# MatrixPlayer/face_alignment_cvpr_2012

Measured on NVIDIA B200. Metric: face crops/sec (head pose + 10-pt FFD), higher is better.
Workload: dtype f32+int32

## Files before the change

face_alignment_cvpr_2012_b200/csrc/device_forest.h:

```cpp
#pragma once
#include <cstdint>
#include <string>
#include <vector>

#include "model.h"

namespace crf {

constexpr int kRowStride = 128;
typedef uint32_t stack_t;
constexpr bool kStack16 = sizeof(stack_t) == 2;
constexpr int kStripArea = kStack16 ? 257 : (1 << 20);
constexpr uint32_t kSumMask = kStack16 ? 0xffffu : 0xffffffffu;
constexpr int kPatch = 31;
constexpr int kHalfPatch = 15;
constexpr int kParts = 10;
constexpr int kMaxList = 128;

struct alignas(32) DevSlot {
  uint16_t a1;
  uint8_t w1, ns1;
  uint16_t hs1;
  uint16_t hl1;
  uint16_t a2;
// ... 5 lines not shown
  uint32_t m1, m2;
  int32_t child;
};
static_assert(sizeof(DevSlot) == 32, "slot must be one 32-byte sector");

struct alignas(16) DevSlot16 { uint32_t r1, r2; int32_t child; uint32_t areas; };
static_assert(sizeof(DevSlot16) == 16, "compact slot is 16 bytes");

constexpr int kWinTile = 8;
constexpr int kWinExtent = 30;
constexpr int kWinRows = kWinTile + kWinExtent;
constexpr int kWinCols = 40;
constexpr int kWinRowBytes = kWinCols * 4;
constexpr int kWinPlaneBytes = kWinRows * kWinRowBytes;
struct alignas(32) DevSlotW {
  uint32_t px1, px2;
  uint32_t yh1, yh2;
  uint32_t m1, m2;
  int32_t child;
  uint32_t tw;
};
static_assert(sizeof(DevSlotW) == 32, "window slot is one 32-byte sector");

struct alignas(32) DevSlotN {
  uint32_t pw1, pw2;
  uint32_t yh1, yh2;
  uint32_t m1, m2;
  int32_t left_thr;
  int32_t right;
};
static_assert(sizeof(DevSlotN) == 32, "internal-node slot is one 32-byte sector");
constexpr int kSlotNChildBits = 22;

struct alignas(16) DevMpLeaf {
  int16_t off[kParts][2];
  float weight;
  uint32_t pad;
};
static_assert(sizeof(DevMpLeaf) == 48, "leaf record is three 16-byte words");

struct PackedForest {
  std::vector<DevSlot> slots;
  std::vector<DevSlot16> slots16;
  std::vector<DevSlotW> slotsw;
  std::vector<DevSlotN> slotsn;
  std::vector<int32_t> nroot;
  int max_extent = 0;
  std::vector<int32_t> roots;
  std::vector<int32_t> forest_base;
  std::vector<int32_t> forest_ntrees;
  std::vector<int32_t> leaf_base;
  std::vector<int32_t> leaf_oid;
  std::vector<float> hp_m;
  std::vector<DevMpLeaf> mp_leaf;
  std::vector<uint16_t> mp_mask;
  int max_depth = 0;
};

struct PackOptions {
  float hp_min_foreground = 0.5f;
  int ffd_min_samples = 2;
  float ffd_min_foreground = 0.5f;
  float ffd_min_pf = 0.25f;
  float ffd_max_variance = 25.f;
};

int pack_forests(const std::vector<const FlatForest*>& forests, ForestKind kind, const PackOptions& opt, PackedForest& out, std::string& err);

inline uint32_t magic_for_area(uint32_t area) { return (uint32_t)((1ull << 31) / area) + 1u; }

}
```

face_alignment_cvpr_2012_b200/csrc/engine.cu:

```cuda
#include <algorithm>
#include <atomic>
#include <cmath>
#include <cstdio>
#include <cstdlib>
#include <cstring>
#include <memory>
#include <sstream>
#include <string>
#include <thread>
#include <unordered_map>
#include <vector>

#include "kernels.cuh"
#include "model.h"

struct crf_model { crf::Model m; };

namespace crf {

thread_local std::string g_last_error;
static int fail(int code, const std::string& msg) { g_last_error = msg; return code; }

#define CU(call)                                                                                          \
  do {                                                                                                    \
// ... 94 lines not shown
};
static ChannelLayout layout_of(const std::vector<int>& sorted_features) {
  ChannelLayout L;
  auto plain = [&](int which) { L.pp.which[L.n_plain] = which; L.pp.plane[L.n_plain] = L.nplanes++; L.n_plain++; };
  for (int f : sorted_features) {
    switch (f) {
      case 0: plain(0); break;
      case 1: L.gabor_first = L.nplanes; L.nplanes += 35; break;
      case 2: plain(1); plain(2); break;
      case 3: plain(3); plain(4); break;
      case 4: plain(6); L.canny = true; break;
      case 5: plain(5); break;
      default: break;
    }
  }
  return L;
}

}

using namespace crf;

struct crf_ctx {
  int device = 0;
  cudaStream_t copy_stream = nullptr;
  cudaEvent_t ev_copied[2] = {nullptr, nullptr}, ev_consumed[2] = {nullptr, nullptr};
  uint8_t* h_stage[2] = {nullptr, nullptr};
  size_t h_stage_bytes[2] = {0, 0};
  crf_options_t opt{};
  int hp_ntrees = 0, mp_ntrees_cfg = 0, num_channels = 38;
  ChannelLayout layout;
  bool full_model = true;
  PackedForest hp, mp;
  Buf d_hp_slotsn, d_mp_slotsn, d_hp_nroot, d_mp_nroot, d_hp_slotsw, d_mp_slotsw, d_hp_slots16, d_mp_slots16, d_hp_slots, d_hp_roots, d_hp_m, d_mp_slots, d_mp_roots, d_mp_mask, d_mp_leaf, d_xs, d_coef[5], d_coef_sep[5];
  int gabor_width[5] = {0, 0, 0, 0, 0};
  ComposeTables ct{};
  struct WorkSet {
    cudaStream_t stream = nullptr;
    Buf d_gabor_scratch, d_gabor_counters;
    Buf d_scaled, d_stacks, d_mag, d_minmax, d_hp_leaf, d_ffd_leaf, d_face_roots, d_face_ntrees, d_votes, d_vote_counts, d_vote_base, d_seg_counts, d_u8planes, d_int32;
    size_t scaled_fs = 0, stack_fs = 0, plane_stride = 0, mag_fs = 0, mag_ps = 0, hp_leaf_fs = 0, ffd_leaf_fs = 0, vote_cap = 0, u8_fs = 0;
    Buf* all[16] = {&d_gabor_scratch, &d_gabor_counters, &d_scaled, &d_stacks, &d_mag, &d_minmax, &d_hp_leaf, &d_ffd_leaf, &d_face_roots, &d_face_ntrees, &d_votes, &d_vote_counts, &d_vote_base,
                    &d_seg_counts, &d_u8planes, &d_int32};
  };
  WorkSet ws[2];
  WorkSet* w = &ws[0];
  Buf d_imgs[2], d_fd, d_faces, d_counters, d_misc;
  crf_counters_t cnt{};
  bool counting = false;
  int traverse_variant = 0;
  int sm_count = 148;
  int win_hp = 0, win_ffd = 0;
  bool win_smem_ok = true;
  int win_tex = 1;
  cudaTextureObject_t tex_hp = 0, tex_mp = 0, tex_hp_wide = 0, tex_mp_wide = 0, tex_hp_n = 0, tex_mp_n = 0;
  int win_fmt = 2;
  int nstreams = 1;
  int gabor_fused = 0;
  int gabor_band = 32;
  int gabor_quant_old = 0;
  int ms_mode = CRF_MS_FAST;
  int ms_variant = 3;
  size_t work_budget = (size_t)64 << 30;
  StageTimer timer;
  unsigned long long haar_cached = 0;
  Buf d_haar_stages, d_haar_weak, d_haar_feats, d_haar_nodes, d_haar_leaves, d_haar_tilt, d_haar_T, d_haar_frames, d_haar_S, d_haar_Q, d_haar_flags, d_haar_list[2], d_haar_rows, d_haar_levels, d_haar_counts, d_haar_cand;
  std::vector<int> haar_split{3, 8};
// ... 294 lines not shown

static int launch_meanshift(crf_ctx* c, const FaceDesc* fd, int nchains, crf_face_t* faces) {
  Span s(c, CRF_STAGE_MEANSHIFT);
  MeanShiftOpt mo{c->opt.ms_kernel_size, c->opt.ms_max_iterations, c->opt.ms_stopping_criteria};
  const int cpc = nchains >= 8192 ? 32 : std::max(1, std::min(8, nchains / 296));
  const dim3 grid((nchains + cpc - 1) / cpc);
  unsigned long long* cnt = c->counting ? c->d_counters.as<unsigned long long>() : nullptr;
  if (c->ms_mode == CRF_MS_FAST) {
    const bool dense = c->w->ffd_leaf_fs >= 65536 || c->w->vote_cap >= 65536;
    if (dense) k_meanshift_fast<512><<<nchains, 512, 0, c->w->stream>>>(fd, nchains, c->w->d_votes.as<DevVote>(), c->w->vote_cap, c->w->d_vote_counts.as<int32_t>(),
                                                                       c->w->d_vote_base.as<int32_t>(), mo, faces, cnt);
    else k_meanshift_fast<128><<<nchains, 128, 0, c->w->stream>>>(fd, nchains, c->w->d_votes.as<DevVote>(), c->w->vote_cap, c->w->d_vote_counts.as<int32_t>(),
                                                                 c->w->d_vote_base.as<int32_t>(), mo, faces, cnt);
    KCHECK(); count_launch(c, CRF_STAGE_MEANSHIFT);
    return CRF_OK;
  }
#define CRF_MS(MINB)                                                                                                                                    \
  k_meanshift<MINB, false><<<grid, kFoldThreads, MsGeom<false>::smem, c->w->stream>>>(fd, nchains, c->w->d_votes.as<DevVote>(), c->w->vote_cap, c->w->d_vote_counts.as<int32_t>(), \
                                                                  c->w->d_vote_base.as<int32_t>(), cpc, mo, faces, cnt)
  if (cpc < 32)
    k_meanshift<3, true><<<grid, kFoldThreads, MsGeom<true>::smem, c->w->stream>>>(fd, nchains, c->w->d_votes.as<DevVote>(), c->w->vote_cap, c->w->d_vote_counts.as<int32_t>(),
                                                                     c->w->d_vote_base.as<int32_t>(), cpc, mo, faces, cnt);
  else if (c->ms_variant == 2) CRF_MS(2); else if (c->ms_variant == 4) CRF_MS(4); else CRF_MS(3);
#undef CRF_MS
  KCHECK(); count_launch(c, CRF_STAGE_MEANSHIFT);
  return CRF_OK;
}

static int launch_votes_meanshift(crf_ctx* c, const FaceDesc* fd, int n, int stride, crf_face_t* faces) {
  {
    Span s(c, CRF_STAGE_VOTES);
    VoteArgs a{};
    a.fd = fd; a.leaf_ids = c->w->d_ffd_leaf.as<int32_t>(); a.leaf_face_stride = c->w->ffd_leaf_fs; a.face_ntrees = c->w->d_face_ntrees.as<int32_t>(); a.stride = stride;
    a.mp_mask = c->d_mp_mask.as<uint16_t>(); a.mp_leaf = c->d_mp_leaf.as<DevMpLeaf>(); a.votes = c->w->d_votes.as<DevVote>(); a.vote_cap = c->w->vote_cap;
    a.seg_counts = c->w->d_seg_counts.as<int32_t>(); a.vote_counts = c->w->d_vote_counts.as<int32_t>(); a.vote_base = c->w->d_vote_base.as<int32_t>(); a.faces = faces;
    CU(cudaMemsetAsync(a.vote_counts, 0, (size_t)n * kParts * 4, c->w->stream));
    k_votes_count<<<dim3(kVoteSegs / 8, n), 256, 0, c->w->stream>>>(a);
    KCHECK();
    k_votes_offsets<<<(n + 127) / 128, 128, 0, c->w->stream>>>(a, n);
    KCHECK();
    k_votes_emit<<<dim3(kVoteSegs / 8, n), 256, 0, c->w->stream>>>(a);
    KCHECK(); count_launch(c, CRF_STAGE_VOTES, 3);
  }
  return launch_meanshift(c, fd, n * kParts, faces);
}

static int run_faces(crf_ctx* c, const FaceDesc* d_fd, int n, int Hmax, const uint8_t* d_imgs, crf_face_t* d_faces, bool headpose_only, int tree_cap,
                     cudaEvent_t imgs_consumed) {
  int rc;
  if ((rc = launch_resize(c, d_fd, n, Hmax, d_imgs))) return rc;
  if (imgs_consumed) CU(cudaEventRecord(imgs_consumed, c->w->stream));
  if ((rc = launch_channels(c, d_fd, n, Hmax, c->layout, false))) return rc;
  if ((rc = launch_traverse(c, d_fd, n, Hmax, true, c->opt.hp_stride, c->d_hp_roots.as<int32_t>(), c->hp_ntrees, c->hp_ntrees, true))) return rc;
  if ((rc = launch_hp_reduce(c, d_fd, n, c->opt.hp_stride, !headpose_only, tree_cap, d_faces))) return rc;
  if (headpose_only) return CRF_OK;
  if ((rc = launch_traverse(c, d_fd, n, Hmax, false, c->opt.ffd_stride, nullptr, 0, tree_cap))) return rc;
  if ((rc = launch_votes_meanshift(c, d_fd, n, c->opt.ffd_stride, d_faces))) return rc;
  return CRF_OK;
}

static int pick_chunk(const crf_ctx* c, int Hmax, bool headpose_only) {
  const size_t np_hp = (size_t)patches_1d(125, c->opt.hp_stride) * patches_1d(Hmax, c->opt.hp_stride);
  const size_t np_ffd = headpose_only ? 0 : (size_t)patches_1d(125, c->opt.ffd_stride) * patches_1d(Hmax, c->opt.ffd_stride);
  const size_t per_face = (size_t)Hmax * 128 + (size_t)(Hmax + 1) * kRowStride * sizeof(stack_t) * c->layout.nplanes +
                          (c->layout.gabor_first >= 0 && !c->gabor_fused ? (size_t)Hmax * 128 * 4 * 35 + 35 * 2 * 4 : 0) + np_hp * c->hp_ntrees * 4 +
                          np_ffd * c->mp_ntrees_cfg * (4 + 3 * sizeof(DevVote)) + (size_t)kMaxList * 4 + 4 +
                          (headpose_only ? 0 : (size_t)kVoteSegs * kParts * 4 + 2 * kParts * 4) + sizeof(FaceDesc) + sizeof(crf_face_t);
// ... 757 lines not shown
    PackedForest pf;
    std::vector<const FlatForest*> fs;
    if (which == 0) fs.push_back(&m->m.hp); else for (auto& f : m->m.jungle) fs.push_back(&f);
    const int rc = pack_forests(fs, which == 0 ? KIND_HEADPOSE : KIND_MULTIPART, po, pf, err);
    if (rc) return fail(rc, err);
    if (pf.slots.size() != pf.slots16.size() || pf.slots.size() != pf.slotsw.size()) return fail(CRF_ERR_STATE, "record arrays differ in length");
    int ext = 0;
    for (size_t i = 0; i < pf.slots.size(); i++) {
      const DevSlot& a = pf.slots[i]; const DevSlot16& b = pf.slots16[i]; const DevSlotW& w = pf.slotsw[i];
      const bool leaf16 = (b.r1 >> 26) & 1u, leafw = (w.tw >> 31) & 1u;
      if ((a.is_leaf != 0) != leaf16 || leaf16 != leafw) return fail(CRF_ERR_STATE, "leaf flags disagree");
      if (a.is_leaf) {
        if (b.child != a.child || (int32_t)w.m2 != a.child || w.child != (int32_t)i || (w.tw & 0xffffu) != 0x7fffu || w.px1 || w.px2 || w.yh1 || w.yh2 || w.m1)
          return fail(CRF_ERR_STATE, "leaf record mismatch");
      } else {
        const int x1 = a.a1 % kRowStride, y1 = a.a1 / kRowStride, x2 = a.a2 % kRowStride, y2 = a.a2 / kRowStride;
        const int h1 = ((a.ns1 - 1) * a.hs1 + a.hl1) / kRowStride, h2 = ((a.ns2 - 1) * a.hs2 + a.hl2) / kRowStride;
        const bool ok16 = (int)(b.r1 & 31) == x1 && (int)((b.r1 >> 5) & 31) == y1 && (int)((b.r1 >> 10) & 31) == a.w1 && (int)((b.r1 >> 15) & 31) == h1 &&
                          (int)((b.r1 >> 20) & 63) == a.ch && (int)(b.r2 & 31) == x2 && (int)((b.r2 >> 5) & 31) == y2 && (int)((b.r2 >> 10) & 31) == a.w2 &&
                          (int)((b.r2 >> 15) & 31) == h2 && (int)((b.r2 >> 20) & 0x3ff) - 256 == a.thr && b.child == a.child &&
                          (b.areas & 0xffff) == (uint32_t)a.w1 * h1 && (b.areas >> 16) == (uint32_t)a.w2 * h2;
        const bool okw = w.px1 == (uint32_t)a.ch * kWinPlaneBytes + x1 * 4u && w.px2 == (uint32_t)a.ch * kWinPlaneBytes + x2 * 4u &&
                         w.yh1 == ((uint32_t)y1 * kWinRowBytes | ((uint32_t)h1 * kWinRowBytes) << 16) && w.yh2 == ((uint32_t)y2 * kWinRowBytes | ((uint32_t)h2 * kWinRowBytes) << 16) &&
                         w.m1 == a.m1 && w.m2 == a.m2 && w.child == a.child && (int)(short)(w.tw & 0xffffu) == a.thr &&
                         ((w.tw >> 16) & 0xffu) == a.w1 * 4u && ((w.tw >> 24) & 0x7fu) == a.w2 * 4u &&
                         a.m1 == magic_for_area((uint32_t)a.w1 * h1) && a.m2 == magic_for_area((uint32_t)a.w2 * h2);
        if (!ok16 || !okw) return fail(CRF_ERR_STATE, "record forms disagree at slot " + std::to_string(i));
        if (a.child <= (int32_t)i || (size_t)a.child + 1 >= pf.slots.size()) return fail(CRF_ERR_STATE, "children are not laid out after their parent");
        ext = std::max(ext, std::max(std::max(x1 + a.w1, y1 + h1), std::max(x2 + a.w2, y2 + h2)));
      }
      checked++;
    }
    if (ext != pf.max_extent) return fail(CRF_ERR_STATE, "max_extent is not the largest rectangle extent");
    if (!pf.nroot.empty()) {
      if (pf.nroot.size() != pf.roots.size()) return fail(CRF_ERR_STATE, "nroot and roots differ in length");
      std::vector<std::pair<int32_t, int32_t>> st;
      for (size_t t = 0; t < pf.roots.size(); t++) {
        st.assign(1, {pf.roots[t], pf.nroot[t]});
        while (!st.empty()) {
          const auto [si, ni] = st.back(); st.pop_back();
          const DevSlot& a = pf.slots[si];
          if (a.is_leaf) { if (ni != ~a.child) return fail(CRF_ERR_STATE, "DevSlotN leaf tag mismatch"); continue; }
          if (ni < 0 || (size_t)ni >= pf.slotsn.size()) return fail(CRF_ERR_STATE, "DevSlotN index out of range");
          const DevSlotN& r = pf.slotsn[ni]; const DevSlotW& w = pf.slotsw[si];
          const int32_t left = (int32_t)((uint32_t)r.left_thr << (32 - kSlotNChildBits)) >> (32 - kSlotNChildBits), thr = r.left_thr >> kSlotNChildBits;
          if ((r.pw1 & 0x3ffffu) != w.px1 || (r.pw2 & 0x3ffffu) != w.px2 || (r.pw1 >> 18) != ((w.tw >> 16) & 0xffu) || (r.pw2 >> 18) != ((w.tw >> 24) & 0x7fu) ||
              r.yh1 != w.yh1 || r.yh2 != w.yh2 || r.m1 != w.m1 || r.m2 != w.m2 || thr != std::min(255, std::max(-256, (int)a.thr)))
            return fail(CRF_ERR_STATE, "DevSlotN test mismatch at slot " + std::to_string(si));
          st.push_back({a.child, left});
          st.push_back({a.child + 1, r.right});
        }
      }
    }
    if (which == 0 && max_extent_hp) *max_extent_hp = ext;
    if (which == 1 && max_extent_ffd) *max_extent_ffd = ext;
  }
  return (int)std::min<long long>(checked, 0x7fffffff);
}

void crf_model_free(crf_model* m) { delete m; }

int crf_device_count(void) {
  int n = 0;
  if (cudaGetDeviceCount(&n) != cudaSuccess) { cudaGetLastError(); return 0; }
  return n;
}

void crf_ctx_destroy(crf_ctx* c) {
  if (!c) return;
  cudaSetDevice(c->device);
  for (auto& w : c->ws) if (w.stream) cudaStreamSynchronize(w.stream);
  if (c->tex_hp) cudaDestroyTextureObject(c->tex_hp);
  if (c->tex_mp) cudaDestroyTextureObject(c->tex_mp);
  if (c->tex_hp_n) cudaDestroyTextureObject(c->tex_hp_n);
  if (c->tex_mp_n) cudaDestroyTextureObject(c->tex_mp_n);
  if (c->tex_hp_wide) cudaDestroyTextureObject(c->tex_hp_wide);
  if (c->tex_mp_wide) cudaDestroyTextureObject(c->tex_mp_wide);
  Buf* all[] = {&c->d_hp_slotsn, &c->d_mp_slotsn, &c->d_hp_nroot, &c->d_mp_nroot, &c->d_hp_slotsw, &c->d_mp_slotsw, &c->d_hp_slots16, &c->d_mp_slots16, &c->d_hp_slots, &c->d_hp_roots, &c->d_hp_m, &c->d_mp_slots, &c->d_mp_roots, &c->d_mp_mask, &c->d_mp_leaf, &c->d_xs, &c->d_coef[0], &c->d_coef[1],
                &c->d_coef[2], &c->d_coef[3], &c->d_coef[4], &c->d_coef_sep[1], &c->d_coef_sep[2], &c->d_coef_sep[3], &c->d_coef_sep[4], &c->d_imgs[0], &c->d_imgs[1], &c->d_fd, &c->d_faces, &c->d_counters, &c->d_misc,
                &c->d_haar_stages, &c->d_haar_weak, &c->d_haar_feats, &c->d_haar_nodes, &c->d_haar_leaves, &c->d_haar_tilt, &c->d_haar_T, &c->d_haar_frames, &c->d_haar_S, &c->d_haar_Q, &c->d_haar_flags, &c->d_haar_list[0],
                &c->d_haar_list[1], &c->d_haar_rows, &c->d_haar_levels, &c->d_haar_counts, &c->d_haar_cand};
  for (Buf* b : all) b->release();
  for (auto& w : c->ws) {
    for (Buf* b : w.all) b->release();
    if (w.stream) cudaStreamDestroy(w.stream);
  }
  c->timer.destroy();
  for (int i = 0; i < 2; i++) { if (c->ev_copied[i]) cudaEventDestroy(c->ev_copied[i]); if (c->ev_consumed[i]) cudaEventDestroy(c->ev_consumed[i]); }
  if (c->copy_stream) cudaStreamDestroy(c->copy_stream);
  for (int i = 0; i < 2; i++) if (c->h_stage[i]) cudaFreeHost(c->h_stage[i]);
  delete c;
}

int crf_ctx_create(const crf_model* m, int device, const crf_options_t* opt, crf_ctx** out) {
  if (!out) return fail(CRF_ERR_ARG, "null argument");
  *out = nullptr;
  static const crf_model no_forests = [] { crf_model e; e.m.features = {0, 1, 2}; e.m.num_channels = 38; return e; }();
  if (!m) m = &no_forests;
  int ndev = 0;
  if (cudaGetDeviceCount(&ndev) != cudaSuccess || ndev <= 0) { cudaGetLastError(); return fail(CRF_ERR_CUDA, "no CUDA device: this library has no CPU fallback"); }
  if (device < 0 || device >= ndev) return fail(CRF_ERR_ARG, "device index out of range");
  const bool full = !m->m.hp.trees.empty() && m->m.jungle.size() == CRF_NUM_POSE_FORESTS;
  if (!m->m.hp.trees.empty() && !m->m.jungle.empty() && m->m.jungle.size() != CRF_NUM_POSE_FORESTS)
    return fail(CRF_ERR_UNSUPPORTED, "the facial-feature jungle must hold 5 pose forests (src/FaceForest.cpp:216-222)");
  CU(cudaSetDevice(device));
  crf_ctx* c = new crf_ctx();
  struct Guard { crf_ctx* c; ~Guard() { if (c) crf_ctx_destroy(c); } } guard{c};
  c->device = device;
  if (opt) c->opt = *opt; else crf_options_default(&c->opt);
  if (c->opt.hp_stride < 1 || c->opt.ffd_stride < 1) return fail(CRF_ERR_ARG, "strides must be >= 1");
  if (const char* v = std::getenv("CRF_TRAVERSE_VARIANT")) c->traverse_variant = (int)std::strtol(v, nullptr, 0);
// ... 21 lines not shown
  }
  for (auto& w : c->ws) CU(cudaStreamCreateWithFlags(&w.stream, cudaStreamNonBlocking));
  CU(cudaStreamCreateWithFlags(&c->copy_stream, cudaStreamNonBlocking));
  for (int i = 0; i < 2; i++) {
    CU(cudaEventCreateWithFlags(&c->ev_copied[i], cudaEventDisableTiming));
    CU(cudaEventCreateWithFlags(&c->ev_consumed[i], cudaEventDisableTiming));
  }
  PackOptions po;
  po.hp_min_foreground = c->opt.hp_min_foreground; po.ffd_min_samples = c->opt.ffd_min_samples; po.ffd_min_foreground = c->opt.ffd_min_foreground;
  po.ffd_min_pf = c->opt.ffd_min_pf; po.ffd_max_variance = c->opt.ffd_max_variance;
  std::string err;
  int rc = CRF_OK;
  if (!m->m.hp.trees.empty() && (rc = pack_forests({&m->m.hp}, KIND_HEADPOSE, po, c->hp, err))) return fail(rc, err);
  std::vector<const FlatForest*> jf;
  for (auto& f : m->m.jungle) jf.push_back(&f);
  if (!jf.empty() && (rc = pack_forests(jf, KIND_MULTIPART, po, c->mp, err))) return fail(rc, err);
  c->hp_ntrees = (int)c->hp.roots.size();
  c->mp_ntrees_cfg = std::max(m->m.mp_ntrees_cfg, 1);
  c->num_channels = m->m.num_channels;
  c->full_model = full;
  c->layout = layout_of(std::vector<int>(m->m.features.begin(), m->m.features.end()));
  if (c->layout.nplanes != c->num_channels) return fail(CRF_ERR_STATE, "feature list and plane count disagree");
  if (c->hp_ntrees > kMaxList || c->mp_ntrees_cfg > kMaxList) return fail(CRF_ERR_UNSUPPORTED, "forest size outside 1..128 trees");
  if ((rc = upload(c->d_hp_slots16, c->hp.slots16, c->w->stream)) || (rc = upload(c->d_mp_slots16, c->mp.slots16, c->w->stream))) return rc;
  if ((rc = upload(c->d_hp_slotsw, c->hp.slotsw, c->w->stream)) || (rc = upload(c->d_mp_slotsw, c->mp.slotsw, c->w->stream))) return rc;
  CU(cudaDeviceGetAttribute(&c->sm_count, cudaDevAttrMultiProcessorCount, device));
  {
    int optin = 0;
    CU(cudaDeviceGetAttribute(&optin, cudaDevAttrMaxSharedMemoryPerBlockOptin, device));
    c->win_smem_ok = optin >= kWinSmemBytes;
  }
  if ((rc = upload(c->d_hp_slots, c->hp.slots, c->w->stream)) || (rc = upload(c->d_hp_roots, c->hp.roots, c->w->stream)) || (rc = upload(c->d_hp_m, c->hp.hp_m, c->w->stream)) ||
      (rc = upload(c->d_mp_slots, c->mp.slots, c->w->stream)) || (rc = upload(c->d_mp_roots, c->mp.roots, c->w->stream)) ||
      (rc = upload(c->d_mp_mask, c->mp.mp_mask, c->w->stream)) || (rc = upload(c->d_mp_leaf, c->mp.mp_leaf, c->w->stream)))
    return rc;
  for (int k = 0; k < 2; k++) {
    const PackedForest& pf = k ? c->mp : c->hp;
    if (pf.slotsn.empty() && pf.nroot.empty()) continue;
    std::vector<int32_t> map(pf.slots.size(), -1);
    for (size_t t = 0; t < pf.roots.size(); t++) map[pf.roots[t]] = pf.nroot[t];
    std::vector<DevSlotN> recs = pf.slotsn;
    if (recs.empty()) recs.emplace_back();
    if ((rc = upload(k ? c->d_mp_slotsn : c->d_hp_slotsn, recs, c->w->stream)) || (rc = upload(k ? c->d_mp_nroot : c->d_hp_nroot, map, c->w->stream))) return rc;
  }
  for (int k = 0; k < 6; k++) {
    cudaResourceDesc rd{}; rd.resType = cudaResourceTypeLinear;
    void* ptrs[6] = {c->d_hp_slotsw.p, c->d_mp_slotsw.p, c->d_hp_slots.p, c->d_mp_slots.p, c->d_hp_slotsn.p, c->d_mp_slotsn.p};
    const size_t counts[6] = {c->hp.slotsw.size(), c->mp.slotsw.size(), c->hp.slots.size(), c->mp.slots.size(),
                              c->d_hp_slotsn.p ? std::max<size_t>(c->hp.slotsn.size(), 1) : 0, c->d_mp_slotsn.p ? std::max<size_t>(c->mp.slotsn.size(), 1) : 0};
    cudaTextureObject_t* objs[6] = {&c->tex_hp, &c->tex_mp, &c->tex_hp_wide, &c->tex_mp_wide, &c->tex_hp_n, &c->tex_mp_n};
    if (counts[k] == 0) continue;
    rd.res.linear.devPtr = ptrs[k];
    rd.res.linear.desc = cudaCreateChannelDesc<uint4>();
    rd.res.linear.sizeInBytes = counts[k] * 32;
    cudaTextureDesc td{}; td.readMode = cudaReadModeElementType;
    CU(cudaCreateTextureObject(objs[k], &rd, &td, nullptr));
  }
  {
    float poseT[6];
    poseT[0] = -2.5; poseT[1] = -0.35; poseT[2] = -0.20; poseT[3] = -poseT[2]; poseT[4] = -poseT[1]; poseT[5] = -poseT[0];
    std::vector<double> xs;
    for (int j = 0; j < 5; j++) {
      c->ct.bin_begin[j] = (int)xs.size();
      const double step = 0.01;
      for (double x = poseT[j]; x < poseT[j + 1]; x += step) xs.push_back(x);
    }
    c->ct.bin_begin[5] = (int)xs.size();
// ... 665 lines not shown
```

face_alignment_cvpr_2012_b200/csrc/kernels.cuh:

```cuda
#pragma once
#include <cuda_runtime.h>
#include <stdint.h>

#include "../../include/crf_b200.h"
#include "device_forest.h"

namespace crf {

struct FaceDesc {
  unsigned long long img_off;
  unsigned long long img_step;
  int bx, by, bw, bh;
  int W, H;
  float scale;
  int pad;
  double scale_x, scale_y;
};

enum { CNT_HP_TESTS = 0, CNT_FFD_TESTS, CNT_HP_TRAV, CNT_FFD_TRAV, CNT_VOTES, CNT_VOTE_PASSES, CNT_NUM };

__device__ __forceinline__ int border101(int p, int len) {
  if (len == 1) return 0;
  while (p < 0 || p >= len) p = p < 0 ? -p : 2 * len - 2 - p;
  return p;
// ... 1601 lines not shown
    for (int j = warp; j < kFoldChains && f0 + j < nfaces; j += kFoldThreads / 32)
      compose_face(s_mean[j], s_var[j], ct, lane, faces + f0 + j, face_roots + (size_t)(f0 + j) * kMaxList, face_ntrees + f0 + j);
}

__global__ void k_area_under_curve(float x1, float x2, double mean, double sd, float* out) {
  double sum = 0;
  const double step = 0.01;
  for (double x = x1; x < x2; x += step) {
    const double t = (x - mean) / sd;
    sum += exp(-0.5 * (t * t)) * step;
  }
  *out = (float)(sum * 1.0 / (sd * sqrt(2 * 3.14159265358979323846)));
}

__global__ void k_compose_only(float headpose, float variance, ComposeTables ct, crf_face_t* face, int32_t* list, int32_t* ntrees) {
  compose_face(headpose, variance, ct, threadIdx.x & 31, face, list, ntrees);
}

__global__ void __launch_bounds__(288) k_compose_batch(const float* __restrict__ headpose, const float* __restrict__ variance, int n, ComposeTables ct,
                                                       crf_face_t* __restrict__ faces, int32_t* __restrict__ lists, int32_t* __restrict__ ntrees) {
  const int i = blockIdx.x * 9 + (threadIdx.x >> 5);
  if (i >= n) return;
  compose_face(headpose[i], variance[i], ct, threadIdx.x & 31, faces + i, lists + (size_t)i * kMaxList, ntrees + i);
}

struct __align__(8) DevVote { short x, y; float w; };

constexpr int kVoteSegs = 128;

struct VoteArgs {
  const FaceDesc* fd;
  const int32_t* leaf_ids; size_t leaf_face_stride;
  const int32_t* face_ntrees; int stride;
  const uint16_t* mp_mask; const DevMpLeaf* mp_leaf;
  DevVote* votes; size_t vote_cap;
  int32_t* seg_counts;
  int32_t* vote_counts;
  int32_t* vote_base;
  crf_face_t* faces;
};

__device__ __forceinline__ void vote_segment(const VoteArgs& a, int f, int seg, int& n, int& k0, int& k1, int& nt, int& ny) {
  const FaceDesc d = a.fd[f];
  nt = a.face_ntrees[f];
  const int nx = (d.W - kPatch + a.stride - 1) / a.stride;
  ny = (d.H - kPatch + a.stride - 1) / a.stride;
  n = max(nx, 0) * max(ny, 0) * nt;
  const int per = (((n + kVoteSegs - 1) / kVoteSegs) + 31) & ~31;
  k0 = min(n, seg * per);
  k1 = min(n, k0 + per);
}

__global__ void __launch_bounds__(256) k_votes_count(VoteArgs a) {
  const int f = blockIdx.y, lane = threadIdx.x & 31, seg = blockIdx.x * 8 + (threadIdx.x >> 5);
  int n, k0, k1, nt, ny;
  vote_segment(a, f, seg, n, k0, k1, nt, ny);
  const int32_t* __restrict__ ids = a.leaf_ids + f * a.leaf_face_stride;
  auto spread5 = [](unsigned x) { return (x * 0x108421u) & 0x01041041u; };
  unsigned lo = 0, hi = 0;
  const bool swar = (k1 - k0 + 31) / 32 <= 63;
  int cnt = 0;
  for (int kb = k0; kb < k1; kb += 128) {
    int id[4];
    unsigned mask[4];
#pragma unroll
    for (int u = 0; u < 4; u++) { const int k = kb + u * 32 + lane; id[u] = k < k1 ? ids[k] : -1; }
#pragma unroll
    for (int u = 0; u < 4; u++) mask[u] = id[u] >= 0 ? (unsigned)__ldg(a.mp_mask + id[u]) : 0u;
    if (swar) {
#pragma unroll
      for (int u = 0; u < 4; u++) { lo += spread5(mask[u] & 31u); hi += spread5(mask[u] >> 5); }
    } else {
#pragma unroll
      for (int p = 0; p < kParts; p++) {
        int c = 0;
#pragma unroll
        for (int u = 0; u < 4; u++) c += __popc(__ballot_sync(0xffffffffu, (mask[u] >> p) & 1u));
        if (lane == p) cnt += c;
      }
    }
  }
  if (swar) {
#pragma unroll
    for (int p = 0; p < kParts; p++) {
      const int c = (int)__reduce_add_sync(0xffffffffu, ((p < 5 ? lo : hi) >> (6 * (p % 5))) & 63u);
      if (lane == p) cnt = c;
    }
  }
  if (lane < kParts) {
    a.seg_counts[((size_t)f * kVoteSegs + seg) * kParts + lane] = cnt;
    if (cnt) atomicAdd(&a.vote_counts[f * kParts + lane], cnt);
  }
}

__global__ void k_votes_offsets(VoteArgs a, int nfaces) {
  const int f = blockIdx.x * blockDim.x + threadIdx.x;
  if (f >= nfaces) return;
  long long run = 0;
  for (int p = 0; p < kParts; p++) { a.vote_base[f * kParts + p] = (int32_t)run; run += a.vote_counts[f * kParts + p]; }
  if (run > (long long)a.vote_cap) {
    for (int p = 0; p < kParts; p++) { a.vote_base[f * kParts + p] = 0; a.vote_counts[f * kParts + p] = -1; }
    a.faces[f].flags |= 4;
  }
}

__global__ void __launch_bounds__(256) k_votes_emit(VoteArgs a) {
  const int f = blockIdx.y, lane = threadIdx.x & 31, seg = blockIdx.x * 8 + (threadIdx.x >> 5);
  int n, k0, k1, nt, ny;
  vote_segment(a, f, seg, n, k0, k1, nt, ny);
  if (k0 >= k1 || a.vote_counts[f * kParts] < 0) return;
  int base[kParts];
  const int32_t* sc = a.seg_counts + (size_t)f * kVoteSegs * kParts;
#pragma unroll
  for (int p = 0; p < kParts; p++) {
    int v = 0;
    for (int s = lane; s < seg; s += 32) v += sc[s * kParts + p];
    base[p] = __reduce_add_sync(0xffffffffu, v) + a.vote_base[f * kParts + p];
  }
  const int32_t* __restrict__ ids = a.leaf_ids + f * a.leaf_face_stride;
  DevVote* __restrict__ fv = a.votes + (size_t)f * a.vote_cap;
  const unsigned m_nt = 0xffffffffu / (unsigned)nt + 1u, m_ny = 0xffffffffu / (unsigned)max(ny, 1) + 1u;
  int leaf_n = 0;
  unsigned mask_n = 0;
  if (k0 + lane < k1) { leaf_n = ids[k0 + lane]; mask_n = __ldg(a.mp_mask + leaf_n); }
  auto spread5 = [](unsigned x) { return (x * 0x108421u) & 0x01041041u; };
  for (int k = k0 + lane; k - lane < k1; k += 32) {
    const int leaf = leaf_n;
    const unsigned mask = mask_n;
    leaf_n = 0; mask_n = 0;
    if (k + 32 < k1) { leaf_n = ids[k + 32]; mask_n = __ldg(a.mp_mask + leaf_n); }
    const unsigned own_lo = spread5(mask & 31u), own_hi = spread5(mask >> 5);
    unsigned lo = own_lo, hi = own_hi;
#pragma unroll
    for (int o = 1; o < 32; o <<= 1) {
      const unsigned nl = __shfl_up_sync(0xffffffffu, lo, o), nh = __shfl_up_sync(0xffffffffu, hi, o);
      if (lane >= o) { lo += nl; hi += nh; }
    }
    const unsigned tot_lo = __shfl_sync(0xffffffffu, lo, 31), tot_hi = __shfl_sync(0xffffffffu, hi, 31);
    if (mask) {
      const unsigned ex_lo = lo - own_lo, ex_hi = hi - own_hi;
      const int patch = nt == 1 ? k : (int)__umulhi((unsigned)k, m_nt);
      const int ix = ny == 1 ? patch : (int)__umulhi((unsigned)patch, m_ny), iy = patch - ix * ny;
      const int cx = ix * a.stride + kHalfPatch, cy = iy * a.stride + kHalfPatch;
      union { uint4 q[3]; DevMpLeaf L; } u;
      const uint4* lp = reinterpret_cast<const uint4*>(a.mp_leaf + leaf);
      u.q[0] = __ldg(lp); u.q[1] = __ldg(lp + 1); u.q[2] = __ldg(lp + 2);
      const DevMpLeaf& L = u.L;
#pragma unroll
      for (int p = 0; p < kParts; p++) {
        if ((mask >> p) & 1u) {
          DevVote v;
          v.x = (short)(L.off[p][0] + cx);
          v.y = (short)(L.off[p][1] + cy);
          v.w = L.weight;
          fv[base[p] + (int)(((p < 5 ? ex_lo : ex_hi) >> (6 * (p % 5))) & 63u)] = v;
        }
      }
    }
#pragma unroll
    for (int p = 0; p < kParts; p++) base[p] += (int)(((p < 5 ? tot_lo : tot_hi) >> (6 * (p % 5))) & 63u);
  }
}

struct MeanShiftOpt { int kernel; int max_iterations; float stopping; };

struct ExpfTable { unsigned long long tab[32]; };
__constant__ ExpfTable c_expf;

__device__ __forceinline__ float expf_glibc(float x, const unsigned long long* __restrict__ tab) {
  const double N = 32.0;
  const double InvLn2N = 0x1.71547652b82fep+0 * N;
  const double C0 = 0x1.c6af84b912394p-5 / N / N / N, C1 = 0x1.ebfce50fac4f3p-3 / N / N, C2 = 0x1.62e42ff0c52d6p-1 / N;
  const double xd = (double)x;
  if (!(xd > -103.0)) return xd != xd ? x : 0.f;
  if (xd > 88.0) return __int_as_float(0x7f800000);
  const double z = InvLn2N * xd;
  const double kd = rint(z);
  const long long ki = (long long)kd;
  const double r = z - kd;
  const double s = __longlong_as_double((long long)(tab[ki & 31] + ((unsigned long long)ki << 47)));
  const double zz = fma(C0, r, C1);
  const double r2 = r * r;
  double y = fma(C2, r, 1.0);
  y = fma(zz, r2, y);
  return (float)(y * s);
}

__device__ __forceinline__ void vote_terms(const DevVote q, bool first_pass, float mx, float my, float lamda, const unsigned long long* __restrict__ tab,
                                           float& w, float& wx, float& wy) {
  if (first_pass) {
    w = q.w;
  } else {
    const float dx = mx - (float)q.x, dy = my - (float)q.y;
// ... 231 lines not shown
```

face_alignment_cvpr_2012_b200/csrc/pack.cc:

```cpp
#include <algorithm>
#include <deque>

#include "../../include/crf_b200.h"
#include "device_forest.h"

namespace crf {

int pack_forests(const std::vector<const FlatForest*>& forests, ForestKind kind, const PackOptions& opt, PackedForest& out, std::string& err) {
  out = PackedForest();
  for (const FlatForest* f : forests) {
    out.forest_base.push_back((int32_t)out.roots.size());
    out.forest_ntrees.push_back((int32_t)f->trees.size());
    for (const FlatTree& t : f->trees) {
      if (t.nodes.empty()) { err = "empty tree"; return CRF_ERR_FORMAT; }
      const int32_t leaf_base = (int32_t)out.leaf_oid.size();
      out.leaf_base.push_back(leaf_base);
      out.max_depth = t.max_depth > out.max_depth ? t.max_depth : out.max_depth;
      const size_t nleaves = kind == KIND_HEADPOSE ? t.hp_leaves.size() : t.mp_leaves.size();
      out.leaf_oid.resize(leaf_base + nleaves);
      if (kind == KIND_HEADPOSE) {
        out.hp_m.resize(leaf_base + nleaves);
        for (size_t l = 0; l < nleaves; l++) {
          const HpLeaf& L = t.hp_leaves[l];
          out.leaf_oid[leaf_base + l] = L.object_id;
          float m = -1.f;
          if (L.foreground > opt.hp_min_foreground) {
            m = 0;
            for (int j = 0; j < 5; j++) m += L.labels[j] * j;
            m /= (L.nsamples * L.foreground);
            if (!(m >= 0.f)) m = __builtin_nanf("");
          }
          out.hp_m[leaf_base + l] = m;
        }
      } else {
        out.mp_leaf.resize(leaf_base + nleaves);
        out.mp_mask.resize(leaf_base + nleaves);
        for (size_t l = 0; l < nleaves; l++) {
          const MpLeaf& L = t.mp_leaves[l];
          out.leaf_oid[leaf_base + l] = L.object_id;
          DevMpLeaf d{};
          uint16_t mask = 0;
          for (int i = 0; i < kParts; i++) {
            if (L.offset[i][0] < -32768 || L.offset[i][0] > 32767 || L.offset[i][1] < -32768 || L.offset[i][1] > 32767) {
              err = "leaf offset does not fit int16"; return CRF_ERR_UNSUPPORTED;
            }
            d.off[i][0] = (int16_t)L.offset[i][0];
            d.off[i][1] = (int16_t)L.offset[i][1];
            float min_pf = opt.ffd_min_pf;
            if (i == 0 || i == 7) min_pf *= 1.5;
            if (L.foreground > opt.ffd_min_foreground && L.prob_foreground[i] > min_pf && L.variance[i] < opt.ffd_max_variance &&
                L.samples > opt.ffd_min_samples)
              mask |= (uint16_t)(1u << i);
          }
          d.weight = L.foreground;
          out.mp_leaf[leaf_base + l] = d;
          out.mp_mask[leaf_base + l] = mask;
        }
      }
      const int32_t base = (int32_t)out.slots.size();
      out.roots.push_back(base);
      std::vector<int32_t> slot_of(t.nodes.size(), -1);
      std::vector<int32_t> n_of(t.nodes.size(), 0);
      auto tag = [&](int32_t ni) {
        if (t.nodes[ni].leaf >= 0) n_of[ni] = ~(leaf_base + t.nodes[ni].leaf);
        else { n_of[ni] = (int32_t)out.slotsn.size(); out.slotsn.emplace_back(); }
      };
      tag(0);
      out.nroot.push_back(n_of[0]);
      std::deque<int32_t> q;
      out.slots.emplace_back();
      slot_of[0] = base;
      q.push_back(0);
      while (!q.empty()) {
        const int32_t ni = q.front();
        q.pop_front();
        const FlatNode& n = t.nodes[ni];
        DevSlot s{};
        if (n.leaf >= 0) {
          s.is_leaf = 1;
          s.child = leaf_base + n.leaf;
        } else {
          if (n.left < 0 || n.right < 0 || n.left >= (int32_t)t.nodes.size() || n.right >= (int32_t)t.nodes.size()) { err = "dangling child"; return CRF_ERR_FORMAT; }
          const int32_t pair = (int32_t)out.slots.size();
          out.slots.emplace_back();
          out.slots.emplace_back();
          slot_of[n.left] = pair;
          slot_of[n.right] = pair + 1;
          q.push_back(n.left);
          q.push_back(n.right);
// ... 71 lines not shown
```

Baseline: 42310.

## Repack vote leaves and compact vote emission through shared-memory owner map

New measurement: 42780 (median of 6 runs). +1.1%, better.

```diff
diff --git a/face_alignment_cvpr_2012_b200/csrc/device_forest.h b/face_alignment_cvpr_2012_b200/csrc/device_forest.h
--- a/face_alignment_cvpr_2012_b200/csrc/device_forest.h
+++ b/face_alignment_cvpr_2012_b200/csrc/device_forest.h
@@ -61,12 +61,11 @@
 static_assert(sizeof(DevSlotN) == 32, "internal-node slot is one 32-byte sector");
 constexpr int kSlotNChildBits = 22;
 
-struct alignas(16) DevMpLeaf {
-  int16_t off[kParts][2];
+struct alignas(8) DevVoteLeaf {
+  uint32_t mask;
   float weight;
-  uint32_t pad;
 };
-static_assert(sizeof(DevMpLeaf) == 48, "leaf record is three 16-byte words");
+static_assert(sizeof(DevVoteLeaf) == 8, "vote leaf record is one 64-bit load");
 
 struct PackedForest {
   std::vector<DevSlot> slots;
@@ -81,8 +80,8 @@
   std::vector<int32_t> leaf_base;
   std::vector<int32_t> leaf_oid;
   std::vector<float> hp_m;
-  std::vector<DevMpLeaf> mp_leaf;
-  std::vector<uint16_t> mp_mask;
+  std::vector<DevVoteLeaf> mp_leaf;
+  std::vector<uint32_t> mp_off;
   int max_depth = 0;
 };
 
diff --git a/face_alignment_cvpr_2012_b200/csrc/engine.cu b/face_alignment_cvpr_2012_b200/csrc/engine.cu
--- a/face_alignment_cvpr_2012_b200/csrc/engine.cu
+++ b/face_alignment_cvpr_2012_b200/csrc/engine.cu
@@ -150,7 +150,7 @@
   ChannelLayout layout;
   bool full_model = true;
   PackedForest hp, mp;
-  Buf d_hp_slotsn, d_mp_slotsn, d_hp_nroot, d_mp_nroot, d_hp_slotsw, d_mp_slotsw, d_hp_slots16, d_mp_slots16, d_hp_slots, d_hp_roots, d_hp_m, d_mp_slots, d_mp_roots, d_mp_mask, d_mp_leaf, d_xs, d_coef[5], d_coef_sep[5];
+  Buf d_hp_slotsn, d_mp_slotsn, d_hp_nroot, d_mp_nroot, d_hp_slotsw, d_mp_slotsw, d_hp_slots16, d_mp_slots16, d_hp_slots, d_hp_roots, d_hp_m, d_mp_slots, d_mp_roots, d_mp_leaf, d_mp_off, d_xs, d_coef[5], d_coef_sep[5];
   int gabor_width[5] = {0, 0, 0, 0, 0};
   ComposeTables ct{};
   struct WorkSet {
@@ -511,7 +511,7 @@
     Span s(c, CRF_STAGE_VOTES);
     VoteArgs a{};
     a.fd = fd; a.leaf_ids = c->w->d_ffd_leaf.as<int32_t>(); a.leaf_face_stride = c->w->ffd_leaf_fs; a.face_ntrees = c->w->d_face_ntrees.as<int32_t>(); a.stride = stride;
-    a.mp_mask = c->d_mp_mask.as<uint16_t>(); a.mp_leaf = c->d_mp_leaf.as<DevMpLeaf>(); a.votes = c->w->d_votes.as<DevVote>(); a.vote_cap = c->w->vote_cap;
+    a.mp_leaf = c->d_mp_leaf.as<DevVoteLeaf>(); a.mp_off = c->d_mp_off.as<uint32_t>(); a.votes = c->w->d_votes.as<DevVote>(); a.vote_cap = c->w->vote_cap;
     a.seg_counts = c->w->d_seg_counts.as<int32_t>(); a.vote_counts = c->w->d_vote_counts.as<int32_t>(); a.vote_base = c->w->d_vote_base.as<int32_t>(); a.faces = faces;
     CU(cudaMemsetAsync(a.vote_counts, 0, (size_t)n * kParts * 4, c->w->stream));
     k_votes_count<<<dim3(kVoteSegs / 8, n), 256, 0, c->w->stream>>>(a);
@@ -1335,6 +1335,23 @@
       checked++;
     }
     if (ext != pf.max_extent) return fail(CRF_ERR_STATE, "max_extent is not the largest rectangle extent");
+    if (which == 1) {
+      size_t l = 0;
+      for (const FlatForest* f : fs)
+        for (const FlatTree& t : f->trees)
+          for (const MpLeaf& L : t.mp_leaves) {
+            if (l >= pf.mp_leaf.size() || pf.mp_off.size() != pf.mp_leaf.size() * kParts)
+              return fail(CRF_ERR_STATE, "vote tables differ in length from the leaves");
+            for (int i = 0; i < kParts; i++) {
+              const uint32_t o = pf.mp_off[l * kParts + i];
+              if ((int16_t)(o & 0xffffu) != L.offset[i][0] || (int16_t)(o >> 16) != L.offset[i][1])
+                return fail(CRF_ERR_STATE, "vote offset mismatch at leaf " + std::to_string(l));
+            }
+            if (std::memcmp(&pf.mp_leaf[l].weight, &L.foreground, sizeof(float)) != 0) return fail(CRF_ERR_STATE, "vote weight mismatch at leaf " + std::to_string(l));
+            l++;
+          }
+      if (l != pf.mp_leaf.size()) return fail(CRF_ERR_STATE, "vote tables differ in length from the leaves");
+    }
     if (!pf.nroot.empty()) {
       if (pf.nroot.size() != pf.roots.size()) return fail(CRF_ERR_STATE, "nroot and roots differ in length");
       std::vector<std::pair<int32_t, int32_t>> st;
@@ -1379,7 +1396,7 @@
   if (c->tex_mp_n) cudaDestroyTextureObject(c->tex_mp_n);
   if (c->tex_hp_wide) cudaDestroyTextureObject(c->tex_hp_wide);
   if (c->tex_mp_wide) cudaDestroyTextureObject(c->tex_mp_wide);
-  Buf* all[] = {&c->d_hp_slotsn, &c->d_mp_slotsn, &c->d_hp_nroot, &c->d_mp_nroot, &c->d_hp_slotsw, &c->d_mp_slotsw, &c->d_hp_slots16, &c->d_mp_slots16, &c->d_hp_slots, &c->d_hp_roots, &c->d_hp_m, &c->d_mp_slots, &c->d_mp_roots, &c->d_mp_mask, &c->d_mp_leaf, &c->d_xs, &c->d_coef[0], &c->d_coef[1],
+  Buf* all[] = {&c->d_hp_slotsn, &c->d_mp_slotsn, &c->d_hp_nroot, &c->d_mp_nroot, &c->d_hp_slotsw, &c->d_mp_slotsw, &c->d_hp_slots16, &c->d_mp_slots16, &c->d_hp_slots, &c->d_hp_roots, &c->d_hp_m, &c->d_mp_slots, &c->d_mp_roots, &c->d_mp_leaf, &c->d_mp_off, &c->d_xs, &c->d_coef[0], &c->d_coef[1],
                 &c->d_coef[2], &c->d_coef[3], &c->d_coef[4], &c->d_coef_sep[1], &c->d_coef_sep[2], &c->d_coef_sep[3], &c->d_coef_sep[4], &c->d_imgs[0], &c->d_imgs[1], &c->d_fd, &c->d_faces, &c->d_counters, &c->d_misc,
                 &c->d_haar_stages, &c->d_haar_weak, &c->d_haar_feats, &c->d_haar_nodes, &c->d_haar_leaves, &c->d_haar_tilt, &c->d_haar_T, &c->d_haar_frames, &c->d_haar_S, &c->d_haar_Q, &c->d_haar_flags, &c->d_haar_list[0],
                 &c->d_haar_list[1], &c->d_haar_rows, &c->d_haar_levels, &c->d_haar_counts, &c->d_haar_cand};
@@ -1467,7 +1484,7 @@
   }
   if ((rc = upload(c->d_hp_slots, c->hp.slots, c->w->stream)) || (rc = upload(c->d_hp_roots, c->hp.roots, c->w->stream)) || (rc = upload(c->d_hp_m, c->hp.hp_m, c->w->stream)) ||
       (rc = upload(c->d_mp_slots, c->mp.slots, c->w->stream)) || (rc = upload(c->d_mp_roots, c->mp.roots, c->w->stream)) ||
-      (rc = upload(c->d_mp_mask, c->mp.mp_mask, c->w->stream)) || (rc = upload(c->d_mp_leaf, c->mp.mp_leaf, c->w->stream)))
+      (rc = upload(c->d_mp_leaf, c->mp.mp_leaf, c->w->stream)) || (rc = upload(c->d_mp_off, c->mp.mp_off, c->w->stream)))
     return rc;
   for (int k = 0; k < 2; k++) {
     const PackedForest& pf = k ? c->mp : c->hp;
diff --git a/face_alignment_cvpr_2012_b200/csrc/kernels.cuh b/face_alignment_cvpr_2012_b200/csrc/kernels.cuh
--- a/face_alignment_cvpr_2012_b200/csrc/kernels.cuh
+++ b/face_alignment_cvpr_2012_b200/csrc/kernels.cuh
@@ -1657,7 +1657,7 @@
   const FaceDesc* fd;
   const int32_t* leaf_ids; size_t leaf_face_stride;
   const int32_t* face_ntrees; int stride;
-  const uint16_t* mp_mask; const DevMpLeaf* mp_leaf;
+  const DevVoteLeaf* mp_leaf; const uint32_t* mp_off;
   DevVote* votes; size_t vote_cap;
   int32_t* seg_counts;
   int32_t* vote_counts;
@@ -1691,7 +1691,7 @@
 #pragma unroll
     for (int u = 0; u < 4; u++) { const int k = kb + u * 32 + lane; id[u] = k < k1 ? ids[k] : -1; }
 #pragma unroll
-    for (int u = 0; u < 4; u++) mask[u] = id[u] >= 0 ? (unsigned)__ldg(a.mp_mask + id[u]) : 0u;
+    for (int u = 0; u < 4; u++) mask[u] = id[u] >= 0 ? __ldg(&a.mp_leaf[id[u]].mask) : 0u;
     if (swar) {
 #pragma unroll
       for (int u = 0; u < 4; u++) { lo += spread5(mask[u] & 31u); hi += spread5(mask[u] >> 5); }
@@ -1730,30 +1730,44 @@
 }
 
 __global__ void __launch_bounds__(256) k_votes_emit(VoteArgs a) {
-  const int f = blockIdx.y, lane = threadIdx.x & 31, seg = blockIdx.x * 8 + (threadIdx.x >> 5);
+  __shared__ uint8_t s_owner[8][kParts * 32];
+  __shared__ int2 s_run[8][kParts];
+  const int f = blockIdx.y, warp = threadIdx.x >> 5, lane = threadIdx.x & 31, seg = blockIdx.x * 8 + warp;
   int n, k0, k1, nt, ny;
   vote_segment(a, f, seg, n, k0, k1, nt, ny);
   if (k0 >= k1 || a.vote_counts[f * kParts] < 0) return;
-  int base[kParts];
+  int base = 0;
   const int32_t* sc = a.seg_counts + (size_t)f * kVoteSegs * kParts;
 #pragma unroll
   for (int p = 0; p < kParts; p++) {
     int v = 0;
     for (int s = lane; s < seg; s += 32) v += sc[s * kParts + p];
-    base[p] = __reduce_add_sync(0xffffffffu, v) + a.vote_base[f * kParts + p];
+    v = __reduce_add_sync(0xffffffffu, v);
+    if (lane == p) base = v + a.vote_base[f * kParts + p];
   }
   const int32_t* __restrict__ ids = a.leaf_ids + f * a.leaf_face_stride;
-  DevVote* __restrict__ fv = a.votes + (size_t)f * a.vote_cap;
+  uint2* __restrict__ fv = reinterpret_cast<uint2*>(a.votes + (size_t)f * a.vote_cap);
+  uint8_t* own = s_owner[warp];
+  int2* run = s_run[warp];
   const unsigned m_nt = 0xffffffffu / (unsigned)nt + 1u, m_ny = 0xffffffffu / (unsigned)max(ny, 1) + 1u;
-  int leaf_n = 0;
-  unsigned mask_n = 0;
-  if (k0 + lane < k1) { leaf_n = ids[k0 + lane]; mask_n = __ldg(a.mp_mask + leaf_n); }
+  const unsigned lt = (1u << lane) - 1u;
+  const int sh = 6 * (lane % 5);
   auto spread5 = [](unsigned x) { return (x * 0x108421u) & 0x01041041u; };
-  for (int k = k0 + lane; k - lane < k1; k += 32) {
+  const uint2* __restrict__ vleaf = reinterpret_cast<const uint2*>(a.mp_leaf);
+  int leaf_n = 0, id_nn = 0;
+  uint2 rec_n = make_uint2(0u, 0u);
+  if (k0 + lane < k1) { leaf_n = ids[k0 + lane]; rec_n = __ldg(vleaf + leaf_n); }
+  if (k0 + 32 + lane < k1) id_nn = ids[k0 + 32 + lane];
+  for (int kb = k0; kb < k1; kb += 32) {
     const int leaf = leaf_n;
-    const unsigned mask = mask_n;
-    leaf_n = 0; mask_n = 0;
-    if (k + 32 < k1) { leaf_n = ids[k + 32]; mask_n = __ldg(a.mp_mask + leaf_n); }
+    const unsigned mask = rec_n.x, wbits = rec_n.y;
+    leaf_n = id_nn;
+    rec_n = kb + 32 + lane < k1 ? __ldg(vleaf + id_nn) : make_uint2(0u, 0u);
+    id_nn = kb + 64 + lane < k1 ? ids[kb + 64 + lane] : 0;
+    const int k = kb + lane;
+    const int patch = nt == 1 ? k : (int)__umulhi((unsigned)k, m_nt);
+    const int ix = ny == 1 ? patch : (int)__umulhi((unsigned)patch, m_ny), iy = patch - ix * ny;
+    const unsigned cxy = (unsigned)(ix * a.stride + kHalfPatch) | (unsigned)(iy * a.stride + kHalfPatch) << 16;
     const unsigned own_lo = spread5(mask & 31u), own_hi = spread5(mask >> 5);
     unsigned lo = own_lo, hi = own_hi;
 #pragma unroll
@@ -1762,28 +1776,42 @@
       if (lane >= o) { lo += nl; hi += nh; }
     }
     const unsigned tot_lo = __shfl_sync(0xffffffffu, lo, 31), tot_hi = __shfl_sync(0xffffffffu, hi, 31);
-    if (mask) {
-      const unsigned ex_lo = lo - own_lo, ex_hi = hi - own_hi;
-      const int patch = nt == 1 ? k : (int)__umulhi((unsigned)k, m_nt);
-      const int ix = ny == 1 ? patch : (int)__umulhi((unsigned)patch, m_ny), iy = patch - ix * ny;
-      const int cx = ix * a.stride + kHalfPatch, cy = iy * a.stride + kHalfPatch;
-      union { uint4 q[3]; DevMpLeaf L; } u;
-      const uint4* lp = reinterpret_cast<const uint4*>(a.mp_leaf + leaf);
-      u.q[0] = __ldg(lp); u.q[1] = __ldg(lp + 1); u.q[2] = __ldg(lp + 2);
-      const DevMpLeaf& L = u.L;
-#pragma unroll
-      for (int p = 0; p < kParts; p++) {
-        if ((mask >> p) & 1u) {
-          DevVote v;
-          v.x = (short)(L.off[p][0] + cx);
-          v.y = (short)(L.off[p][1] + cy);
-          v.w = L.weight;
-          fv[base[p] + (int)(((p < 5 ? ex_lo : ex_hi) >> (6 * (p % 5))) & 63u)] = v;
-        }
-      }
-    }
-#pragma unroll
-    for (int p = 0; p < kParts; p++) base[p] += (int)(((p < 5 ? tot_lo : tot_hi) >> (6 * (p % 5))) & 63u);
+    const unsigned ex_lo = lo - own_lo, ex_hi = hi - own_hi;
+#pragma unroll
+    for (int p = 0; p < kParts; p++)
+      if ((mask >> p) & 1u) own[p * 32 + (int)(((p < 5 ? ex_lo : ex_hi) >> (6 * (p % 5))) & 63u)] = (uint8_t)lane;
+    const int t = lane < kParts ? (int)(((lane < 5 ? tot_lo : tot_hi) >> sh) & 63u) : 0;
+    int P = t;
+#pragma unroll
+    for (int o = 1; o < 16; o <<= 1) {
+      const int np = __shfl_up_sync(0xffffffffu, P, o);
+      if (lane >= o) P += np;
+    }
+    const int T = __shfl_sync(0xffffffffu, P, kParts - 1);
+    P -= t;
+    const unsigned live = __ballot_sync(0xffffffffu, t > 0);
+    if (t > 0) run[__popc(live & lt)] = make_int2(base - P, 32 * lane - P);
+    base += t;
+    __syncwarp();
+    for (int j0 = 0; j0 < T; j0 += 32) {
+      const int j = j0 + lane;
+      const unsigned starts = __reduce_or_sync(0xffffffffu, t > 0 && P >= j0 && P < j0 + 32 ? 1u << (P - j0) : 0u);
+      const int before = __popc(__ballot_sync(0xffffffffu, t > 0 && P < j0));
+      int owner = 0;
+      int2 r = make_int2(0, 0);
+      if (j < T) {
+        r = run[before + __popc(starts & (lt | (1u << lane))) - 1];
+        owner = own[j + r.y];
+      }
+      const int lf = __shfl_sync(0xffffffffu, leaf, owner);
+      const unsigned c = __shfl_sync(0xffffffffu, cxy, owner), wb = __shfl_sync(0xffffffffu, wbits, owner);
+      if (j < T) {
+        const unsigned off = __ldg(a.mp_off + (size_t)lf * kParts + ((j + r.y) >> 5));
+        const unsigned xy = __byte_perm(off + c, off + (c & 0xffff0000u), 0x7610);
+        fv[j + r.x] = make_uint2(xy, wb);
+      }
+    }
+    __syncwarp();
   }
 }
 
diff --git a/face_alignment_cvpr_2012_b200/csrc/pack.cc b/face_alignment_cvpr_2012_b200/csrc/pack.cc
--- a/face_alignment_cvpr_2012_b200/csrc/pack.cc
+++ b/face_alignment_cvpr_2012_b200/csrc/pack.cc
@@ -34,27 +34,23 @@
         }
       } else {
         out.mp_leaf.resize(leaf_base + nleaves);
-        out.mp_mask.resize(leaf_base + nleaves);
+        out.mp_off.resize((leaf_base + nleaves) * kParts);
         for (size_t l = 0; l < nleaves; l++) {
           const MpLeaf& L = t.mp_leaves[l];
           out.leaf_oid[leaf_base + l] = L.object_id;
-          DevMpLeaf d{};
-          uint16_t mask = 0;
+          uint32_t mask = 0;
           for (int i = 0; i < kParts; i++) {
             if (L.offset[i][0] < -32768 || L.offset[i][0] > 32767 || L.offset[i][1] < -32768 || L.offset[i][1] > 32767) {
               err = "leaf offset does not fit int16"; return CRF_ERR_UNSUPPORTED;
             }
-            d.off[i][0] = (int16_t)L.offset[i][0];
-            d.off[i][1] = (int16_t)L.offset[i][1];
+            out.mp_off[(leaf_base + l) * kParts + i] = (uint16_t)L.offset[i][0] | (uint32_t)(uint16_t)L.offset[i][1] << 16;
             float min_pf = opt.ffd_min_pf;
             if (i == 0 || i == 7) min_pf *= 1.5;
             if (L.foreground > opt.ffd_min_foreground && L.prob_foreground[i] > min_pf && L.variance[i] < opt.ffd_max_variance &&
                 L.samples > opt.ffd_min_samples)
-              mask |= (uint16_t)(1u << i);
+              mask |= 1u << i;
           }
-          d.weight = L.foreground;
-          out.mp_leaf[leaf_base + l] = d;
-          out.mp_mask[leaf_base + l] = mask;
+          out.mp_leaf[leaf_base + l] = DevVoteLeaf{mask, L.foreground};
         }
       }
       const int32_t base = (int32_t)out.slots.size();
```
